# p768lwy3/torecsys

Hardware: AMD Instinct MI355X
Metric: CTR samples/sec fwd+bwd (DeepFM, 39 fields x dim 64) (higher is better)
Workload: dtype bf16; 1 GPU; BASELINE.json configs[1]: DeepFM 39 Criteo-shaped fields, MLP [400,400,400], 1000000 total rows, embed_dim 64, batch 65536, uniform indices, uniform field sizes; global_batch=65536, rows=1000000, parallelism=single, microbatches=1, optimizer=none, hipgraph=True, hipgraph_input_sets=1, hipgraph_steps_per_replay=4, fused_lookup_fm=True

## Files before the change

### include/trs_abi.h

```cpp
#ifndef TRS_ABI_H_
#define TRS_ABI_H_

#include <stddef.h>
#include <stdint.h>

#ifdef __cplusplus
extern "C" {
#endif

#define TRS_ABI_VERSION 3

enum { TRS_F32 = 0, TRS_BF16 = 1 };
enum { TRS_I64 = 0, TRS_I32 = 1 };
enum {
  TRS_OK = 0,
  TRS_EINVAL = -1,
  TRS_EDTYPE = -2,
  TRS_ESHAPE = -3,
  TRS_EALIGN = -4,
  TRS_ELAUNCH = -5,
  TRS_EWORKSPACE = -6
};

typedef void* trs_stream_t;
// ... 25 lines not shown
                       int32_t* err_flag, trs_stream_t stream);

size_t trs_scatter_workspace_bytes(int64_t BN, int32_t N, int32_t E, int32_t dtype);
int trs_scatter_rows(const void* g_rows, int64_t g_rows_batch_stride, const void* g_fm, int32_t g_fm_cols,
                     const float* fm_sum, const void* table, const int32_t* row_start,
                     const int32_t* perm, int64_t BN, int64_t V, int32_t E, int32_t N, int32_t dtype,
                     int64_t padding_row, void* grad_table, void* workspace, size_t ws_bytes,
                     trs_stream_t stream);

int trs_scatter_rows_first(const void* g_rows, int64_t g_rows_batch_stride, const void* g_fm, int32_t g_fm_cols,
                           const float* fm_sum,
                           const void* table, const int32_t* row_start, const int32_t* perm, int64_t BN, int64_t V,
                           int32_t E, int32_t N, int32_t dtype, int64_t padding_row, void* grad_table,
                           const void* g_first, void* grad_first, void* workspace, size_t ws_bytes,
                           trs_stream_t stream);

#define TRS_OPT_ROWWISE 16
int trs_scatter_rows_update(const void* g_rows, int64_t g_rows_batch_stride, const void* g_fm, int32_t g_fm_cols,
                            const float* fm_sum, void* table, const int32_t* row_start, const int32_t* perm,
                            int64_t BN, int64_t V, int32_t E, int32_t N, int32_t dtype, int64_t padding_row,
                            int32_t optimizer, float lr, const float* lr_dev, float eps, float beta1, float beta2,
                            float* state, float* state2, void* workspace, size_t ws_bytes, trs_stream_t stream);

int trs_scatter_rows_update_mapped(const void* g_rows, void* table, const int32_t* row_map, const int32_t* row_start,
                                   const int32_t* perm, int64_t K, int64_t U, int64_t V, int32_t E, int32_t dtype,
                                   int32_t optimizer, float lr, const float* lr_dev, float eps, float beta1, float beta2,
                                   float* state, float* state2, void* workspace, size_t ws_bytes, trs_stream_t stream);

int trs_adam_step_size(int64_t* step, const float* lr_dev, double beta1, double beta2, float* step_size_dev,
                       trs_stream_t stream);
// ... 438 lines not shown
```

### torecsys_amd/_abi.py

```python
from __future__ import annotations

import ctypes
import os
import threading
from ctypes import c_char_p, c_int32, c_int64, c_size_t, c_void_p

import torch

_HERE = os.path.dirname(os.path.abspath(__file__))
LIB_PATH = os.environ.get("TRS_LIB_PATH") or os.path.join(_HERE, "libtrs_hip.so")

TRS_F32, TRS_BF16 = 0, 1
TRS_I64, TRS_I32 = 0, 1

_P, _I32, _I64, _SZ, _F32 = c_void_p, c_int32, c_int64, c_size_t, ctypes.c_float

_OPTIMIZER_TAIL = [_I32, _F32, _P, _F32, _F32, _F32, _P, _P, _P, _SZ, _P]

SIGNATURES = {
    "trs_version": (c_int32, []),
    "trs_last_error_string": (c_char_p, []),
    "trs_rowdot_fwd": (c_int32, [_P, _P, _P, _I64, _I32, _I32, _P, _P]),
    "trs_rowdot_bwd_workspace_bytes": (_SZ, [_I64, _I32]),
    "trs_rowdot_bwd": (c_int32, [_P, _P, _P, _I64, _I32, _I32, _P, _P, _P, _P, _SZ, _P]),
# ... 53 lines not shown
    "trs_rows_gemm": (c_int32, [_P, _I64, _I32, _P, _I32, _I32, _I32, _P, _P, _SZ, _P]),
    "trs_afm_bwd_workspace_bytes": (_SZ, [_I64, _I32, _I32, _I32]),
    "trs_pack_columns": (c_int32, [_P, _P, _I32, _I32, _I64, _P, _I32, _P]),
    "trs_mark_timestamp": (c_int32, [_P, _I32, _P]),
    "trs_wall_clock_khz": (_I64, []),
    "trs_gather_rows": (c_int32, [_P, _I64, _I32, _I32, _P, _I32, _P, _I64, _I32, _P, _P, _P]),
    "trs_gather_rows_tables": (c_int32, [_P, _P, _I32, _I32, _P, _I32, _I64, _I32, _P, _P, _P]),
    "trs_fa_gather_rows": (c_int32, [_P, _I64, _I32, _I32, _P, _I32, _P, _I64, _I32, _P, _P, _P]),
    "trs_csr_workspace_bytes": (_SZ, [_I64, _I64]),
    "trs_csr_build": (c_int32, [_P, _I32, _P, _I64, _I32, _I64, _P, _P, _P, _SZ, _P, _P]),
    "trs_csr_build_skip": (c_int32, [_P, _I32, _P, _I64, _I32, _I64, _I64, _P, _P, _P, _SZ, _P, _P]),
    "trs_scatter_workspace_bytes": (_SZ, [_I64, _I32, _I32, _I32]),
    "trs_scatter_rows": (c_int32, [_P, _I64, _P, _I32, _P, _P, _P, _P, _I64, _I64, _I32, _I32, _I32, _I64, _P, _P, _SZ, _P]),
    "trs_scatter_rows_first": (c_int32, [_P, _I64, _P, _I32, _P, _P, _P, _P, _I64, _I64, _I32, _I32, _I32, _I64, _P, _P, _P, _P,
                                         _SZ, _P]),
    "trs_scatter_rows_update": (c_int32, [_P, _I64, _P, _I32, _P, _P, _P, _P, _I64, _I64, _I32, _I32, _I32, _I64,
                                          *_OPTIMIZER_TAIL]),
    "trs_scatter_rows_update_mapped": (c_int32, [_P, _P, _P, _P, _P, _I64, _I64, _I64, _I32, _I32, *_OPTIMIZER_TAIL]),
    "trs_adam_step_size": (c_int32, [_P, _P, ctypes.c_double, ctypes.c_double, _P, _P]),
    "trs_compact_rows_slots": (_I64, [_I64]),
    "trs_compact_rows": (c_int32, [_P, _I64, _P, _I64, _P, _P]),
    "trs_compact_rows_dense_workspace_bytes": (_SZ, [_I64]),
    "trs_compact_rows_dense": (c_int32, [_P, _I64, _P, _P, _P, _SZ, _P]),
    "trs_embed_fm": (c_int32, [_P, _I64, _I32, _I32, _P, _I32, _P, _I64, _I32, _P, _P, _P, _P, _P, _P, _P]),
    "trs_embed_fm_fields": (c_int32, [_P, _I64, _I32, _I32, _P, _I32, _P, _I64, _I32, _P, _P, _P, _P, _P, _P, _P]),
    "trs_bag_pool_fwd": (c_int32, [_P, _I64, _I32, _I32, _P, _I32, _I64, _I32, _I32, _P, _P, _P, _P]),
    "trs_scatter_argmax_workspace_bytes": (_SZ, [_I64, _I32]),
    "trs_scatter_rows_argmax": (c_int32, [_P, _P, _P, _P, _I64, _I64, _I32, _I32, _I32, _I64, _P, _P, _SZ, _P]),
    "trs_bag_pool_masked_fwd": (c_int32, [_P, _I64, _I32, _I32, _P, _I32, _I64, _I32, _I32, _I64, _P, _P, _P, _P, _P, _P]),
    "trs_scatter_weighted_workspace_bytes": (_SZ, [_I64, _I32]),
# ... 330 lines not shown
```

### torecsys_amd/csrc/scatter.hip

```cpp
#include <algorithm>

#include "trs_common.hpp"

namespace trs {

constexpr int SCAN_THREADS = 256;
constexpr int SCAN_ITEMS = 16;
constexpr int SCAN_TILE = SCAN_THREADS * SCAN_ITEMS;
constexpr int LONG_ROW = 64;
constexpr int LONG_ROW_ELEM = 32;
constexpr int LONG_CHUNK = 256;
constexpr int ELEM_SPLIT = 2048;

template <typename IdxT, bool SKIP = false>
__global__ __launch_bounds__(256) void csr_count_kernel(const IdxT* __restrict__ idx,
                                                        const int64_t* __restrict__ offsets, int64_t BN, int N,
                                                        int64_t V, int32_t* __restrict__ count,
                                                        int32_t* __restrict__ slot, int32_t* __restrict__ err_flag,
                                                        const int32_t* __restrict__ gate, int64_t skip_row = -1) {
  constexpr int U = 4;
  if (gate != nullptr && *gate == 0) return;
  const unsigned n_items = (unsigned)BN, uN = (unsigned)N;
  const unsigned stride = gridDim.x * blockDim.x;
  for (unsigned p0 = blockIdx.x * blockDim.x + threadIdx.x; p0 < n_items; p0 += stride * U) {
// ... 546 lines not shown
            } else {
#pragma unroll
              for (int k = 0; k < VE; ++k) gsum[k] += gf[k];
            }
          } else {
#pragma unroll
            for (int k = 0; k < VE; ++k) acc[k] += gf[k];
          }
        }
      }
    }
  }
}

template <typename T, int LOG2L, bool HAS_G, bool HAS_FM, bool HAS_F1 = false, bool SCAL = false, int CHF = 2,
          bool RW = false>
__global__ __launch_bounds__(256) void scatter_rows_group_kernel(
    const uint4* __restrict__ g_rows, const uint4* __restrict__ g_fm, const float* __restrict__ fm_sum,
    const uint4* __restrict__ table, const int32_t* __restrict__ row_start, const int32_t* __restrict__ perm,
    int64_t V, int N, int64_t gbs, int64_t padding_row, uint4* __restrict__ grad,
    int32_t* __restrict__ long_rows , RowSink sink, FmSrc fs, const T* __restrict__ g_first = nullptr,
    T* __restrict__ grad_first = nullptr) {
  constexpr int L = 1 << LOG2L;
  constexpr int VE = Vec16<T>::VE;
  const int lane_v = threadIdx.x & (L - 1);
  const int64_t groups = ((int64_t)gridDim.x * blockDim.x) >> LOG2L;
  int64_t r = ((int64_t)blockIdx.x * blockDim.x + threadIdx.x) >> LOG2L;
  int nbeg = 0, nend = 0;
  if (r < V) { nbeg = row_start[r]; nend = row_start[r + 1]; }
  for (; r < V; r += groups) {
    const int beg = nbeg, end = nend;
// ... 15 lines not shown
      continue;
    }
    float f1 = 0.f;
    if (r != padding_row) {
      accumulate_bucket<T, LOG2L, HAS_G, HAS_FM, (HAS_FM ? CHF : 4), HAS_F1, SCAL>(acc, gsum, g_rows, g_fm, fm_sum, perm, beg,
                                                                                end, 1, N, gbs, lane_v, fs, g_first, &f1);
      if (HAS_FM && fm_sum != nullptr && end > beg) {
        float w[VE];
        Vec16<T>::unpack(wraw, w);
#pragma unroll
        for (int k = 0; k < VE; ++k) acc[k] = fmaf(-w[k], gsum[SCAL ? 0 : k], acc[k]);
      }
    }
    sink_vec<T, RW, LOG2L>(sink, grad, sink_row(sink, r) * L + lane_v, acc, end > beg && r != padding_row);
    if (HAS_F1 && lane_v == 0) grad_first[r] = from_f32<T>(f1);
  }
}

template <typename T, int LOG2L, bool HAS_G, bool RW = false>
__global__ __launch_bounds__(256, 8) void scatter_rows_fm1_kernel(
    const uint4* __restrict__ g_rows, const uint4* __restrict__ tg, const T* __restrict__ g1,
    const uint4* __restrict__ table, const int32_t* __restrict__ row_start, const int32_t* __restrict__ perm, int V,
    unsigned N, unsigned rcpN , int padding_row, uint4* __restrict__ grad,
    int32_t* __restrict__ long_rows , RowSink sink) {
  constexpr int L = 1 << LOG2L;
  constexpr int VE = Vec16<T>::VE;
  constexpr int CH = 2;
  const unsigned lane_v = threadIdx.x & (L - 1);
  const int groups = (int)(((int64_t)gridDim.x * blockDim.x) >> LOG2L);
  int r = (int)(((int64_t)blockIdx.x * blockDim.x + threadIdx.x) >> LOG2L);
  int nbeg = 0, nend = 0;
  if (r < V) { nbeg = row_start[r]; nend = row_start[r + 1]; }
  for (; r < V; r += groups) {
    const int beg = nbeg, end = nend;
    if (r + groups < V) { nbeg = row_start[r + groups]; nend = row_start[r + groups + 1]; }
    const uint4 wraw = table[(unsigned)r * L + lane_v];
    float acc[VE], gsum = 0.f;
#pragma unroll
    for (int k = 0; k < VE; ++k) acc[k] = 0.f;
// ... 39 lines not shown
          if (HAS_G) Vec16<T>::unpack(gv[c], x);
          Vec16<T>::unpack(tv[c], t);
#pragma unroll
          for (int k = 0; k < VE; ++k) acc[k] += HAS_G ? x[k] + t[k] : t[k];
          gsum += gs[c];
        }
      }
      if (end > beg) {
        float w[VE];
        Vec16<T>::unpack(wraw, w);
#pragma unroll
        for (int k = 0; k < VE; ++k) acc[k] = fmaf(-w[k], gsum, acc[k]);
      }
    }
    sink_vec<T, RW, LOG2L>(sink, grad, sink_row(sink, r) * L + lane_v, acc, end > beg && live);
  }
}

template <typename T>
__global__ __launch_bounds__(256) void scatter_first_long_kernel(const T* __restrict__ g_first,
                                                                 const int32_t* __restrict__ row_start,
                                                                 const int32_t* __restrict__ perm,
                                                                 const int32_t* __restrict__ long_rows,
                                                                 T* __restrict__ grad_first) {
  const int nlong = long_rows[0];
  const int lane = threadIdx.x & 63;
  const int wid = (blockIdx.x * blockDim.x + threadIdx.x) >> 6, nwaves = (gridDim.x * blockDim.x) >> 6;
  for (int i = wid; i < nlong; i += nwaves) {
    if (long_rows[2 + 2 * i] != 0) continue;
    const int64_t r = long_rows[1 + 2 * i];
// ... 1 lines not shown
    float acc = 0.f;
    constexpr int U = 4;
    for (int q = beg + lane; q < end; q += 64 * U) {
      int pp[U];
#pragma unroll
      for (int u = 0; u < U; ++u) pp[u] = (q + 64 * u) < end ? perm[q + 64 * u] : -1;
#pragma unroll
      for (int u = 0; u < U; ++u)
        if (pp[u] >= 0) acc += to_f32(g_first[pp[u]]);
    }
    acc = group_sum_down<64>(acc);
    if (lane == 0) grad_first[r] = from_f32<T>(acc);
  }
}

template <typename T, int LOG2L, bool HAS_G, bool HAS_FM, bool SCAL = false, bool RW = false>
__global__ __launch_bounds__(256) void scatter_long_rows_kernel(
    const uint4* __restrict__ g_rows, const uint4* __restrict__ g_fm, const float* __restrict__ fm_sum,
    const uint4* __restrict__ table, const int32_t* __restrict__ row_start, const int32_t* __restrict__ perm, int N,
    int64_t gbs, uint4* __restrict__ grad, const int32_t* __restrict__ long_rows, float* __restrict__ scratch,
    RowSink sink, FmSrc fs) {
  constexpr int L = 1 << LOG2L;
  constexpr int VE = Vec16<T>::VE;
  constexpr int G = 64 / L;
  const int lane = threadIdx.x & 63;
  const int lane_v = lane & (L - 1);
  const int grp = lane >> LOG2L;
  const int nlong = long_rows[0];
  const int waves = gridDim.x * (blockDim.x >> 6);
  for (int i = blockIdx.x * (blockDim.x >> 6) + (threadIdx.x >> 6); i < nlong; i += waves) {
    const int64_t r = long_rows[1 + 2 * i];
    const int c = long_rows[2 + 2 * i];
    const int rbeg = row_start[r], rend = row_start[r + 1];
    const int beg = rbeg + c * LONG_CHUNK, end = rend < beg + LONG_CHUNK ? rend : beg + LONG_CHUNK;
    const bool single = rend - rbeg <= LONG_CHUNK;
    float acc[VE], gsum[VE];
// ... 9 lines not shown
      for (int k = 0; k < (SCAL ? 1 : VE); ++k) gsum[k] += __shfl_xor(gsum[k], m, 64);
    }
    if (SCAL) {
#pragma unroll
      for (int k = 1; k < VE; ++k) gsum[k] = gsum[0];
    }
    if (grp == 0) {
      if (single) {
        if (HAS_FM && fm_sum != nullptr) {
          float w[VE];
          Vec16<T>::unpack(table[r * L + lane_v], w);
#pragma unroll
          for (int k = 0; k < VE; ++k) acc[k] = fmaf(-w[k], gsum[k], acc[k]);
        }
        sink_vec<T, RW, LOG2L>(sink, grad, sink_row(sink, r) * L + lane_v, acc, true);
      } else {
        float* sa = scratch + ((size_t)i * 2) * (L * VE) + lane_v * VE;
#pragma unroll
        for (int k = 0; k < VE; ++k) { sa[k] = acc[k]; sa[L * VE + k] = gsum[k]; }
      }
    }
  }
}

template <typename T, int LOG2L, bool HAS_FM, bool RW = false>
__global__ __launch_bounds__(256) void scatter_long_rows_finish_kernel(
    const float* __restrict__ fm_sum, const uint4* __restrict__ table, const int32_t* __restrict__ row_start,
    uint4* __restrict__ grad, const int32_t* __restrict__ long_rows, const float* __restrict__ scratch, RowSink sink) {
  constexpr int L = 1 << LOG2L;
  constexpr int VE = Vec16<T>::VE;
  const int lane_v = threadIdx.x & (L - 1);
  const int nlong = long_rows[0];
  const int groups = (gridDim.x * blockDim.x) >> LOG2L;
  for (int i = (blockIdx.x * blockDim.x + threadIdx.x) >> LOG2L; i < nlong; i += groups) {
    if (long_rows[2 + 2 * i] != 0) continue;
    const int64_t r = long_rows[1 + 2 * i];
    const int len = row_start[r + 1] - row_start[r];
    if (len <= LONG_CHUNK) continue;
    const int nch = (len + LONG_CHUNK - 1) / LONG_CHUNK;
    float acc[VE], gsum[VE];
#pragma unroll
    for (int k = 0; k < VE; ++k) { acc[k] = 0.f; gsum[k] = 0.f; }
    constexpr int U = 8;
// ... 15 lines not shown
          gsum[4 * k] += vg[u][k].x; gsum[4 * k + 1] += vg[u][k].y; gsum[4 * k + 2] += vg[u][k].z; gsum[4 * k + 3] += vg[u][k].w;
        }
    }
    for (; c < nch; ++c) {
      const float* sa = scratch + ((size_t)(i + c) * 2) * (L * VE) + lane_v * VE;
#pragma unroll
      for (int k = 0; k < VE; ++k) { acc[k] += sa[k]; gsum[k] += sa[L * VE + k]; }
    }
    if (HAS_FM && fm_sum != nullptr) {
      float w[VE];
      Vec16<T>::unpack(table[r * L + lane_v], w);
#pragma unroll
      for (int k = 0; k < VE; ++k) acc[k] = fmaf(-w[k], gsum[k], acc[k]);
    }
    sink_vec<T, RW, LOG2L>(sink, grad, sink_row(sink, r) * L + lane_v, acc, true);
  }
}

template <typename T>
__global__ __launch_bounds__(256) void build_tg_kernel(const uint4* __restrict__ g_fm, const float* __restrict__ fm_sum,
                                                       uint4* __restrict__ tg, int64_t B, int L,
                                                       int32_t* __restrict__ zero_a, int32_t* __restrict__ zero_b) {
  constexpr int VE = Vec16<T>::VE;
  if (zero_a != nullptr && blockIdx.x == 0 && threadIdx.x == 0) { *zero_a = 0; *zero_b = 0; }
  const int64_t total = B * L, stride = (int64_t)gridDim.x * blockDim.x;
  for (int64_t t = (int64_t)blockIdx.x * blockDim.x + threadIdx.x; t < total; t += stride) {
    const int64_t b = t / L;
    const int lv = (int)(t - b * L);
    const uint4 gv = g_fm[t];
    float g[VE], o[VE];
// ... 182 lines not shown
struct WalkJob {
  const void* g_rows = nullptr;
  int64_t gbs = 0;
  const void* g_fm = nullptr;
  int g_fm_cols = 0;
  const float* fm_sum = nullptr;
  const void* table = nullptr;
  const int32_t* row_start = nullptr;
  const int32_t* perm = nullptr;
  int64_t B = 0, V = 0;
  int E = 0, N = 0;
  int64_t padding_row = -1;
  void* out = nullptr;
  const void* g_first = nullptr;
  void* grad_first = nullptr;
  int32_t* long_rows = nullptr;
  bool zero_in_build = false;
  int32_t* split_count = nullptr;
  void* tg = nullptr;
  float* scratch = nullptr;
  RowSink sink = GRAD_SINK;
  hipStream_t s = nullptr;
  const char* who = "scatter_rows";
};

template <typename T, int LOG2L, bool RW>
static void scatter_group_launch(const WalkJob& j) {
  const int L = 1 << LOG2L;
  hipStream_t s = j.s;
  FmSrc fs{nullptr, nullptr, 0, 0};
// ... 5 lines not shown
      uint4* gvec = (uint4*)j.tg + j.B * L;
      hipLaunchKernelGGL((build_tg1_kernel<T>), dim3(stream_grid(j.B * L, 256, 4096)), dim3(256), 0, s,
                         (const T*)j.g_fm, j.fm_sum, (uint4*)j.tg, gvec, j.B, L, zero_a, j.split_count);
      fs = FmSrc{(const uint4*)j.tg, gvec, L, 1};
      fs.g1 = j.g_fm;
      scal = j.g_first == nullptr;
    } else {
      hipLaunchKernelGGL((build_tg_kernel<T>), dim3(stream_grid(j.B * L, 256, 4096)), dim3(256), 0, s,
                         (const uint4*)j.g_fm, j.fm_sum, (uint4*)j.tg, j.B, L, zero_a, j.split_count);
      fs = FmSrc{(const uint4*)j.tg, (const uint4*)j.tg + L, 2 * L, 2 * L};
    }
    fm = j.tg;
  }
  const int grid = stream_grid(j.V * L, 256, 256 * 32);
  const bool hg = j.g_rows != nullptr, hf = fm != nullptr;
#define TRS_SC_TAIL(HG, HF, SC)                                                                                 \
  do {                                                                                                          \
    hipLaunchKernelGGL((scatter_long_rows_kernel<T, LOG2L, HG, HF, SC, RW>), dim3(2048), dim3(256), 0, s,            \
                       (const uint4*)j.g_rows, (const uint4*)fm, j.fm_sum, (const uint4*)j.table, j.row_start,  \
                       j.perm, j.N, j.gbs, (uint4*)j.out, j.long_rows, j.scratch, j.sink, fs);                  \
    hipLaunchKernelGGL((scatter_long_rows_finish_kernel<T, LOG2L, HF, RW>), dim3(64), dim3(256), 0, s, j.fm_sum,    \
                       (const uint4*)j.table, j.row_start, (uint4*)j.out, j.long_rows, j.scratch, j.sink);      \
  } while (0)
#define TRS_SC(HG, HF)                                                                                          \
  do {                                                                                                          \
    if (j.g_first != nullptr)                                                                                   \
      hipLaunchKernelGGL((scatter_rows_group_kernel<T, LOG2L, HG, HF, true>), dim3(grid), dim3(256), 0, s,       \
                         (const uint4*)j.g_rows, (const uint4*)fm, j.fm_sum, (const uint4*)j.table, j.row_start, \
                         j.perm, j.V, j.N, j.gbs, j.padding_row, (uint4*)j.out, j.long_rows, j.sink, fs,        \
                         (const T*)j.g_first, (T*)j.grad_first);                                                \
    else                                                                                                        \
      hipLaunchKernelGGL((scatter_rows_group_kernel<T, LOG2L, HG, HF, false, false, 2, RW>), dim3(grid), dim3(256), 0, s,             \
                         (const uint4*)j.g_rows, (const uint4*)fm, j.fm_sum, (const uint4*)j.table, j.row_start, \
                         j.perm, j.V, j.N, j.gbs, j.padding_row, (uint4*)j.out, j.long_rows, j.sink, fs);       \
    TRS_SC_TAIL(HG, HF, false);                                                                                 \
  } while (0)
#define TRS_SCS(HG, CHF_)                                                                                       \
  do {                                                                                                          \
    hipLaunchKernelGGL((scatter_rows_group_kernel<T, LOG2L, HG, true, false, true, CHF_, RW>), dim3(grid), dim3(256), 0, s, \
                       (const uint4*)j.g_rows, (const uint4*)fm, j.fm_sum, (const uint4*)j.table, j.row_start,  \
                       j.perm, j.V, j.N, j.gbs, j.padding_row, (uint4*)j.out, j.long_rows, j.sink, fs);         \
    TRS_SC_TAIL(HG, true, true);                                                                                \
  } while (0)
  const bool lean = scal && (j.B * j.N) * (int64_t)L < ((int64_t)1 << 31) && j.V * (int64_t)L < ((int64_t)1 << 31) &&
                    j.N >= 2 && (j.B * j.N) * (int64_t)j.N < ((int64_t)1 << 32) && j.gbs == j.N;
  if (lean) {
    const unsigned rcpN = (unsigned)((((uint64_t)1 << 32) + (unsigned)j.N - 1) / (unsigned)j.N);
    if (hg)
      hipLaunchKernelGGL((scatter_rows_fm1_kernel<T, LOG2L, true, RW>), dim3(grid), dim3(256), 0, s, (const uint4*)j.g_rows,
                         (const uint4*)j.tg, (const T*)fs.g1, (const uint4*)j.table, j.row_start, j.perm, (int)j.V,
                         (unsigned)j.N, rcpN, (int)j.padding_row, (uint4*)j.out, j.long_rows, j.sink);
    else
      hipLaunchKernelGGL((scatter_rows_fm1_kernel<T, LOG2L, false, RW>), dim3(grid), dim3(256), 0, s, (const uint4*)j.g_rows,
                         (const uint4*)j.tg, (const T*)fs.g1, (const uint4*)j.table, j.row_start, j.perm, (int)j.V,
                         (unsigned)j.N, rcpN, (int)j.padding_row, (uint4*)j.out, j.long_rows, j.sink);
    if (hg) TRS_SC_TAIL(true, true, true);
    else TRS_SC_TAIL(false, true, true);
  } else if (scal) {
    if (hg) TRS_SCS(true, 2);
    else TRS_SCS(false, 2);
  } else if (hg && hf) TRS_SC(true, true);
  else if (hg) TRS_SC(true, false);
  else TRS_SC(false, true);
#undef TRS_SC
#undef TRS_SCS
#undef TRS_SC_TAIL
  if (j.g_first != nullptr)
    hipLaunchKernelGGL((scatter_first_long_kernel<T>), dim3(64), dim3(256), 0, s, (const T*)j.g_first, j.row_start,
                       j.perm, j.long_rows, (T*)j.grad_first);
}

static int walk_lanes(const WalkJob& j, int elem_bytes) {
  const int lg = log2_lanes(j.E * elem_bytes);
  const bool scal = j.g_fm_cols == 1 && j.E > 1 && j.fm_sum != nullptr;
  const bool al = aligned16(j.g_rows) && (scal || aligned16(j.g_fm)) && aligned16(j.table) && aligned16(j.out) &&
                  aligned16(j.fm_sum);
  return al ? lg : -1;
}

template <typename T>
// ... 173 lines not shown
  TRS_REQUIRE(j.g_rows || j.g_fm, TRS_EINVAL, "scatter_rows: need g_rows and/or g_fm");
  TRS_REQUIRE((j.fm_sum == nullptr) || (j.g_fm && j.table), TRS_EINVAL, "scatter_rows: fm_sum needs g_fm and table");
  TRS_REQUIRE(j.g_fm == nullptr || j.g_fm_cols == j.E || (j.g_fm_cols == 1 && j.fm_sum != nullptr), TRS_EINVAL,
              "scatter_rows: g_fm_cols %d (E = %d full rows, or 1 = constant along E with fm_sum)", j.g_fm_cols, j.E);
  if (j.gbs <= 0) j.gbs = j.N;
  TRS_REQUIRE(j.gbs >= j.N, TRS_EINVAL, "scatter_rows: g_rows_batch_stride %lld < N", (long long)j.gbs);
  TRS_REQUIRE(j.V > 0 && j.E > 0 && j.N > 0 && BN >= 0, TRS_EINVAL, "scatter_rows: bad size");
  TRS_REQUIRE(dtype == TRS_F32 || dtype == TRS_BF16, TRS_EDTYPE, "scatter_rows: dtype %d", dtype);
  TRS_REQUIRE(ws_bytes >= trs_scatter_workspace_bytes(BN, j.N, j.E, dtype), TRS_EWORKSPACE,
              "scatter_rows: workspace %zu < %zu", ws_bytes, trs_scatter_workspace_bytes(BN, j.N, j.E, dtype));
  TRS_REQUIRE(BN % j.N == 0, TRS_EINVAL, "scatter_rows: B*N=%lld not a multiple of N=%d", (long long)BN, j.N);
  const int lg = walk_lanes(j, dtype_size(dtype));
  TRS_REQUIRE(j.sink.mode != 4 || lg >= 0, TRS_ESHAPE,
              "%s: row-wise Adagrad needs rows of 1, 2, 4 .. 64 whole 16-byte vectors behind 16-byte aligned pointers "
              "(E = %d, %d bytes per value)", j.who, j.E, dtype_size(dtype));
  j.B = BN / j.N;
  j.long_rows = (int32_t*)workspace;
  j.tg = (char*)workspace + long_row_queue_bytes(BN);
  j.scratch = (float*)((char*)j.tg + align_up((size_t)j.B * 2 * j.E * dtype_size(dtype), 256));
  j.split_count = j.long_rows + 1 + (BN / LONG_ROW_ELEM + 2);
  j.zero_in_build = lg >= 0 && j.g_fm != nullptr && j.fm_sum != nullptr;
  if (!j.zero_in_build) hipLaunchKernelGGL(zero_two_i32_kernel, dim3(1), dim3(64), 0, j.s, j.long_rows, j.split_count);
  return dtype == TRS_F32 ? scatter_launch<float>(j, lg) : scatter_launch<bf16_t>(j, lg);
}

extern "C" int trs_scatter_rows_first(const void* g_rows, int64_t g_rows_batch_stride, const void* g_fm, int32_t g_fm_cols,
                                      const float* fm_sum, const void* table, const int32_t* row_start,
                                      const int32_t* perm, int64_t BN, int64_t V, int32_t E, int32_t N, int32_t dtype,
                                      int64_t padding_row, void* grad_table, const void* g_first, void* grad_first,
                                      void* workspace, size_t ws_bytes, trs_stream_t stream) {
  TRS_REQUIRE(g_first && grad_first, TRS_EINVAL, "scatter_rows_first: NULL first-order pointer");
  return scatter_rows_impl(WalkJob{.g_rows = g_rows, .gbs = g_rows_batch_stride, .g_fm = g_fm, .g_fm_cols = g_fm_cols,
                                   .fm_sum = fm_sum, .table = table, .row_start = row_start, .perm = perm, .V = V, .E = E,
                                   .N = N, .padding_row = padding_row, .out = grad_table, .g_first = g_first,
                                   .grad_first = grad_first, .sink = GRAD_SINK, .s = (hipStream_t)stream},
                           BN, dtype, workspace, ws_bytes);
}

extern "C" int trs_scatter_rows(const void* g_rows, int64_t g_rows_batch_stride, const void* g_fm, int32_t g_fm_cols,
                                const float* fm_sum,
                                const void* table, const int32_t* row_start, const int32_t* perm, int64_t BN, int64_t V,
                                int32_t E, int32_t N, int32_t dtype, int64_t padding_row, void* grad_table,
                                void* workspace, size_t ws_bytes, trs_stream_t stream) {
  return scatter_rows_impl(WalkJob{.g_rows = g_rows, .gbs = g_rows_batch_stride, .g_fm = g_fm, .g_fm_cols = g_fm_cols,
                                   .fm_sum = fm_sum, .table = table, .row_start = row_start, .perm = perm, .V = V, .E = E,
                                   .N = N, .padding_row = padding_row, .out = grad_table, .sink = GRAD_SINK,
                                   .s = (hipStream_t)stream},
                           BN, dtype, workspace, ws_bytes);
}

// ... 76 lines not shown
```

### torecsys_amd/functional.py

```python
from __future__ import annotations

import ctypes
import os
from typing import List, Optional, Sequence, Tuple

import torch
from torch.autograd import Function
from torch.autograd.function import once_differentiable

from . import _abi
from ._abi import call, index_dtype_code, ptr, require_device, size_query, stream_ptr, value_dtype_code

CHECK_INDICES = os.environ.get("TRS_CHECK_INDICES", "0") not in ("", "0")


def _as_index(idx: torch.Tensor) -> torch.Tensor:
    idx = idx.rename(None) if idx.has_names() else idx
    if idx.dtype not in (torch.int64, torch.int32):
        if idx.dtype.is_floating_point or idx.dtype == torch.bool:
            raise TypeError(f"indices must be an integer tensor, got {idx.dtype}")
        idx = idx.long()
    return idx.contiguous()


# ... 267 lines not shown
    return grad


def scatter_rows_first(rb: RowBuckets, like_table: torch.Tensor, like_first: torch.Tensor, g_first: torch.Tensor,
                       g_rows: Optional[torch.Tensor] = None, g_bcast: Optional[torch.Tensor] = None,
                       fm_sum: Optional[torch.Tensor] = None, padding_row: int = -1
                       ) -> Tuple[torch.Tensor, torch.Tensor]:
    V, E = like_table.shape
    grad = torch.empty_like(like_table)
    gfirst = torch.empty_like(like_first)
    ws_bytes = size_query("trs_scatter_workspace_bytes", rb.BN, rb.N, E, value_dtype_code(like_table))
    ws = torch.empty(ws_bytes, dtype=torch.uint8, device=like_table.device)
    call("trs_scatter_rows_first", ptr(g_rows), 0, ptr(g_bcast), _bcast_cols(g_bcast, E), ptr(fm_sum),
         ptr(like_table if fm_sum is not None else None), ptr(rb.row_start), ptr(rb.perm), rb.BN, V, E, rb.N,
         value_dtype_code(like_table), padding_row, ptr(grad), ptr(g_first), ptr(gfirst), ptr(ws), ws_bytes, stream_ptr())
    return grad, gfirst


def _adam_step_dev(opt, table: torch.Tensor, key) -> torch.Tensor:
    step, step_size = opt.step_tensors(table, key)
    call("trs_adam_step_size", ptr(step), ptr(opt.lr_tensor(table.device)), float(opt.beta1), float(opt.beta2),
         ptr(step_size), stream_ptr())
    return step_size


TRS_OPT_ROWWISE = 16


def _sink_args(opt, table: torch.Tensor, key, operands=()):
    capturable = getattr(opt, "capturable", False)
# ... 876 lines not shown
    if idx.dim() != 2:
        raise ValueError(f"indices must be (B, N), got shape {tuple(idx.shape)}")
    if padding_idx is not None and padding_idx < 0:
        padding_idx = weight.shape[0] + padding_idx
    emb, fm, first = _EmbedFM.apply(weight, idx, offsets, first_weight, want_emb, opt, False, padding_idx)
    return (emb if want_emb else None), fm, (first if first_weight is not None else None)


def embed_fm_fields(weight: torch.Tensor, first_weight: torch.Tensor, idx: torch.Tensor,
                    offsets: Optional[torch.Tensor] = None, opt=None
                    ) -> Tuple[torch.Tensor, torch.Tensor, torch.Tensor]:
    idx = _as_index(idx)
    if idx.dim() != 2:
        raise ValueError(f"indices must be (B, N), got shape {tuple(idx.shape)}")
    return _EmbedFM.apply(weight, idx, offsets, first_weight, True, opt, True)


class _FMLayer(Function):
    @staticmethod
    def forward(ctx, x):
        require_device(x)
        x = x.contiguous()
        B, N, E = x.shape
        fm = torch.empty(B, E, dtype=x.dtype, device=x.device)
        fm_sum = torch.empty(B, E, dtype=torch.float32, device=x.device)
        call("trs_fm_fwd", ptr(x), B, N, E, value_dtype_code(x), ptr(fm), ptr(fm_sum), stream_ptr())
        ctx.save_for_backward(x, fm_sum)
        return fm

    @staticmethod
# ... 2540 lines not shown
```

### torecsys_amd/inputs.py

```python
from __future__ import annotations

import os
from collections import namedtuple
from typing import Dict, List, Optional, Union

import torch
import torch.nn as nn

from . import functional as F_


def _strip(t: torch.Tensor) -> torch.Tensor:
    return t.rename(None) if t.has_names() else t


def _check_embedding_kwargs(kwargs: dict):
    if kwargs.get("max_norm") is not None:
        raise NotImplementedError("torecsys_amd: nn.Embedding(max_norm=...) is not supported")
    if kwargs.get("scale_grad_by_freq"):
        raise NotImplementedError("torecsys_amd: nn.Embedding(scale_grad_by_freq=True) is not supported")
    if kwargs.get("sparse"):
        raise NotImplementedError("torecsys_amd: nn.Embedding(sparse=True) is not supported (dense gradient only)")


# ... 464 lines not shown
        self.num_fields = num_fields
        self.transforms = transforms
        self.length = 1

    def forward(self, inputs: torch.Tensor) -> torch.Tensor:
        inputs = _strip(inputs)
        if inputs.dim() == 2:
            inputs = inputs.unsqueeze(dim=-1)
        if self.transforms:
            inputs = self.transforms(inputs)
        inputs.names = ('B', 'N', 'E',)
        return inputs


PAIR_FIRST_ORDER = os.environ.get("TRS_PAIR_FIRST_ORDER", "0") == "1"


def _on_hip(t: torch.Tensor) -> bool:
    return t.is_cuda


STACKED_ONE_LAUNCH = os.environ.get("TRS_STACKED_ONE_LAUNCH", "1") not in ("", "0")
LOOKUP_STREAMS = int(os.environ.get("TRS_LOOKUP_STREAMS", "1") or 0)
_SIDE_LOOKUPS = (SingleIndexEmbedding, MultiIndicesEmbedding, MultiIndicesFieldAwareEmbedding)


class Inputs(BaseInput):

    def __init__(self, schema: Union[Dict[str, nn.Module], None]):
        super().__init__()
        self.schema = schema if schema is not None else {}
        for k, emb_fn in self.schema.items():
            self.add_module(k, emb_fn)
        self.length = None

    def _first_order_partner(self, key: str) -> Optional[str]:
        a = self.schema[key]
        if not PAIR_FIRST_ORDER:
            return None
        if type(a) is not MultiIndicesEmbedding or not a.fuse_fm or a.flatten or a.padding_idx is not None:
            return None
        if getattr(a, 'fused_optimizer', None) is not None or not a.embedding.weight.is_cuda:
            return None
        wa = a.embedding.weight
        if (wa.shape[1] * wa.element_size()) % 16 != 0:
            return None
        for k, f in self.schema.items():
            if k == key or type(f) is not MultiIndicesEmbedding:
                continue
            if (f.embed_size != 1 or f.flatten or f.fuse_fm or f.padding_idx is not None
                    or getattr(f, 'fused_optimizer', None) is not None):
                continue
            wf = f.embedding.weight
            if (tuple(f.schema.inputs) != tuple(a.schema.inputs) or wf.shape[0] != wa.shape[0] or wf.dtype != wa.dtype
                    or wf.device != wa.device or wf.requires_grad != wa.requires_grad):
                continue
            same = self._same_layout.get((key, k))
# ... 71 lines not shown
                else:
                    cols = [v.unsqueeze(-1) if v.dim() == 1 else v for v in raw]
                    inp = cols[0] if len(cols) == 1 else torch.cat(cols, dim=1)
                packed[names] = inp
            args[k] = [inp]
            if emb_fn.__class__.__name__ in ('SequenceIndicesEmbedding', 'SequenceIndexEmbedding'):
                args[k].append(inputs[emb_fn.schema.lengths])
            elif emb_fn.__class__.__name__ in ('RaggedListIndicesEmbedding', 'RaggedMultiListIndicesEmbedding'):
                args[k].append(inputs[emb_fn.schema.offsets])
                args[k].append(None if emb_fn.schema.weights is None else inputs[emb_fn.schema.weights])
            elif getattr(emb_fn.schema, 'weights', None) is not None:
                args[k].append(inputs[emb_fn.schema.weights])
        side_keys, first_lookup = [], True
        for k in args:
            emb_fn = self.schema[k]
            plain = (type(emb_fn) in _SIDE_LOOKUPS and k not in partner.values()
                     and isinstance(args[k][0], torch.Tensor) and args[k][0].is_cuda)
            if plain and not first_lookup and LOOKUP_STREAMS:
                side_keys.append(k)
            first_lookup = first_lookup and not plain
        joins = []
        def side_lookups():
            for k in side_keys:
                emb_fn, idx_t = self.schema[k], args[k][0]
                out, ev, side = F_.run_on_side(idx_t.device, "lookup", lambda: emb_fn(idx_t))
                idx_t.record_stream(side)
                joins.append((ev, out))
                outputs[k] = out

        with F_.defer_prefetch():
            if LOOKUP_STREAMS == 2:
                side_lookups()
            for k in args:
                if k in outputs or k in side_keys:
                    continue
                emb_fn, inp_args = self.schema[k], args[k]
                feat_key = next((f for f, w in partner.items() if w == k), None)
                if feat_key is not None:
                    feat_fn = self.schema[feat_key]
                    idx = inp_args[0].rename(None) if inp_args[0].has_names() else inp_args[0]
                    if idx.dim() != 2 or idx.shape[1] != emb_fn.offsets.numel():
                        raise ValueError(f'inputs must be (B, {emb_fn.offsets.numel()}), got {tuple(idx.shape)}')
                    out, fm, first = F_.embed_fm_fields(emb_fn.embedding.weight, feat_fn.embedding.weight, idx,
                                                        emb_fn.offsets)
                    out._trs_fused_fm = (fm, out._version)
                    out.names = ('B', 'N', 'E',)
                    first.names = ('B', 'N', 'E',)
                    outputs[k] = out
                    outputs[feat_key] = first
                else:
                    outputs[k] = emb_fn(*inp_args)
            if LOOKUP_STREAMS != 2:
                side_lookups()
        if joins:
            main = F_._abi.current_stream_of(joins[0][1].device)
            for ev, out in joins:
                main.wait_event(ev)
                extra = [t[0] for t in (getattr(out, a, None) for a in ('_trs_fused_fm', '_trs_fused_ipn')) if t is not None]
                for t in [out] + extra:
# ... 22 lines not shown
```

Before: 67.40 million samples/s.

## Pair first-order table with FM embedding and fuse its gradient into the scatter walk

Adds a new default-on path (TRS_PAIR_FIRST_ORDER_WALK) that pairs the first-order linear table with the FM embedding lookup. The forward runs the first-order gather on a side stream, and the backward uses one scatter walk that writes both the embedding gradient and the first-order gradient. It relies on the FM output gradient and the first-order gradient being the same broadcast column, so the per-row sum already computed for the FM term also serves as the first-order gradient. This removes a separate scatter pass over the first-order table. In exchange it adds template variants and a narrower eligibility check that falls back when the gradients do not share storage.

```diff
diff --git a/include/trs_abi.h b/include/trs_abi.h
--- a/include/trs_abi.h
+++ b/include/trs_abi.h
@@ -63,6 +63,12 @@
                            int32_t E, int32_t N, int32_t dtype, int64_t padding_row, void* grad_table,
                            const void* g_first, void* grad_first, void* workspace, size_t ws_bytes,
                            trs_stream_t stream);
+
+int trs_scatter_rows_first_same(const void* g_rows, int64_t g_rows_batch_stride, const void* g_fm, int32_t g_fm_cols,
+                                const float* fm_sum, const void* table, const int32_t* row_start, const int32_t* perm,
+                                int64_t BN, int64_t V, int32_t E, int32_t N, int32_t dtype, int64_t padding_row,
+                                void* grad_table, void* grad_first, void* workspace, size_t ws_bytes,
+                                trs_stream_t stream);
 
 #define TRS_OPT_ROWWISE 16
 int trs_scatter_rows_update(const void* g_rows, int64_t g_rows_batch_stride, const void* g_fm, int32_t g_fm_cols,
diff --git a/torecsys_amd/_abi.py b/torecsys_amd/_abi.py
--- a/torecsys_amd/_abi.py
+++ b/torecsys_amd/_abi.py
@@ -91,6 +91,8 @@
     "trs_scatter_rows": (c_int32, [_P, _I64, _P, _I32, _P, _P, _P, _P, _I64, _I64, _I32, _I32, _I32, _I64, _P, _P, _SZ, _P]),
     "trs_scatter_rows_first": (c_int32, [_P, _I64, _P, _I32, _P, _P, _P, _P, _I64, _I64, _I32, _I32, _I32, _I64, _P, _P, _P, _P,
                                          _SZ, _P]),
+    "trs_scatter_rows_first_same": (c_int32, [_P, _I64, _P, _I32, _P, _P, _P, _P, _I64, _I64, _I32, _I32, _I32, _I64, _P, _P, _P,
+                                              _SZ, _P]),
     "trs_scatter_rows_update": (c_int32, [_P, _I64, _P, _I32, _P, _P, _P, _P, _I64, _I64, _I32, _I32, _I32, _I64,
                                           *_OPTIMIZER_TAIL]),
     "trs_scatter_rows_update_mapped": (c_int32, [_P, _P, _P, _P, _P, _I64, _I64, _I64, _I32, _I32, *_OPTIMIZER_TAIL]),
diff --git a/torecsys_amd/csrc/scatter.hip b/torecsys_amd/csrc/scatter.hip
--- a/torecsys_amd/csrc/scatter.hip
+++ b/torecsys_amd/csrc/scatter.hip
@@ -584,7 +584,7 @@
 }
 
 template <typename T, int LOG2L, bool HAS_G, bool HAS_FM, bool HAS_F1 = false, bool SCAL = false, int CHF = 2,
-          bool RW = false>
+          bool RW = false, bool F1S = false>
 __global__ __launch_bounds__(256) void scatter_rows_group_kernel(
     const uint4* __restrict__ g_rows, const uint4* __restrict__ g_fm, const float* __restrict__ fm_sum,
     const uint4* __restrict__ table, const int32_t* __restrict__ row_start, const int32_t* __restrict__ perm,
@@ -630,15 +630,16 @@
     }
     sink_vec<T, RW, LOG2L>(sink, grad, sink_row(sink, r) * L + lane_v, acc, end > beg && r != padding_row);
     if (HAS_F1 && lane_v == 0) grad_first[r] = from_f32<T>(f1);
-  }
-}
-
-template <typename T, int LOG2L, bool HAS_G, bool RW = false>
+    if (F1S && lane_v == 0) grad_first[r] = from_f32<T>(gsum[0]);
+  }
+}
+
+template <typename T, int LOG2L, bool HAS_G, bool RW = false, bool F1S = false>
 __global__ __launch_bounds__(256, 8) void scatter_rows_fm1_kernel(
     const uint4* __restrict__ g_rows, const uint4* __restrict__ tg, const T* __restrict__ g1,
     const uint4* __restrict__ table, const int32_t* __restrict__ row_start, const int32_t* __restrict__ perm, int V,
     unsigned N, unsigned rcpN , int padding_row, uint4* __restrict__ grad,
-    int32_t* __restrict__ long_rows , RowSink sink) {
+    int32_t* __restrict__ long_rows , RowSink sink, T* __restrict__ grad_first = nullptr) {
   constexpr int L = 1 << LOG2L;
   constexpr int VE = Vec16<T>::VE;
   constexpr int CH = 2;
@@ -708,6 +709,7 @@
       }
     }
     sink_vec<T, RW, LOG2L>(sink, grad, sink_row(sink, r) * L + lane_v, acc, end > beg && live);
+    if (F1S && lane_v == 0) grad_first[r] = from_f32<T>(gsum);
   }
 }
 
@@ -739,12 +741,12 @@
   }
 }
 
-template <typename T, int LOG2L, bool HAS_G, bool HAS_FM, bool SCAL = false, bool RW = false>
+template <typename T, int LOG2L, bool HAS_G, bool HAS_FM, bool SCAL = false, bool RW = false, bool F1S = false>
 __global__ __launch_bounds__(256) void scatter_long_rows_kernel(
     const uint4* __restrict__ g_rows, const uint4* __restrict__ g_fm, const float* __restrict__ fm_sum,
     const uint4* __restrict__ table, const int32_t* __restrict__ row_start, const int32_t* __restrict__ perm, int N,
     int64_t gbs, uint4* __restrict__ grad, const int32_t* __restrict__ long_rows, float* __restrict__ scratch,
-    RowSink sink, FmSrc fs) {
+    RowSink sink, FmSrc fs, T* __restrict__ grad_first = nullptr) {
   constexpr int L = 1 << LOG2L;
   constexpr int VE = Vec16<T>::VE;
   constexpr int G = 64 / L;
@@ -784,6 +786,7 @@
           for (int k = 0; k < VE; ++k) acc[k] = fmaf(-w[k], gsum[k], acc[k]);
         }
         sink_vec<T, RW, LOG2L>(sink, grad, sink_row(sink, r) * L + lane_v, acc, true);
+        if (F1S && lane_v == 0) grad_first[r] = from_f32<T>(gsum[0]);
       } else {
         float* sa = scratch + ((size_t)i * 2) * (L * VE) + lane_v * VE;
 #pragma unroll
@@ -793,10 +796,11 @@
   }
 }
 
-template <typename T, int LOG2L, bool HAS_FM, bool RW = false>
+template <typename T, int LOG2L, bool HAS_FM, bool RW = false, bool F1S = false>
 __global__ __launch_bounds__(256) void scatter_long_rows_finish_kernel(
     const float* __restrict__ fm_sum, const uint4* __restrict__ table, const int32_t* __restrict__ row_start,
-    uint4* __restrict__ grad, const int32_t* __restrict__ long_rows, const float* __restrict__ scratch, RowSink sink) {
+    uint4* __restrict__ grad, const int32_t* __restrict__ long_rows, const float* __restrict__ scratch, RowSink sink,
+    T* __restrict__ grad_first = nullptr) {
   constexpr int L = 1 << LOG2L;
   constexpr int VE = Vec16<T>::VE;
   const int lane_v = threadIdx.x & (L - 1);
@@ -842,6 +846,7 @@
       for (int k = 0; k < VE; ++k) acc[k] = fmaf(-w[k], gsum[k], acc[k]);
     }
     sink_vec<T, RW, LOG2L>(sink, grad, sink_row(sink, r) * L + lane_v, acc, true);
+    if (F1S && lane_v == 0) grad_first[r] = from_f32<T>(gsum[0]);
   }
 }
 
@@ -1054,6 +1059,7 @@
   void* out = nullptr;
   const void* g_first = nullptr;
   void* grad_first = nullptr;
+  bool first_same = false;
   int32_t* long_rows = nullptr;
   bool zero_in_build = false;
   int32_t* split_count = nullptr;
@@ -1089,13 +1095,15 @@
   }
   const int grid = stream_grid(j.V * L, 256, 256 * 32);
   const bool hg = j.g_rows != nullptr, hf = fm != nullptr;
-#define TRS_SC_TAIL(HG, HF, SC)                                                                                 \
+#define TRS_SC_TAIL(HG, HF, SC, F1)                                                                             \
   do {                                                                                                          \
-    hipLaunchKernelGGL((scatter_long_rows_kernel<T, LOG2L, HG, HF, SC, RW>), dim3(2048), dim3(256), 0, s,            \
+    hipLaunchKernelGGL((scatter_long_rows_kernel<T, LOG2L, HG, HF, SC, RW, F1>), dim3(2048), dim3(256), 0, s,   \
                        (const uint4*)j.g_rows, (const uint4*)fm, j.fm_sum, (const uint4*)j.table, j.row_start,  \
-                       j.perm, j.N, j.gbs, (uint4*)j.out, j.long_rows, j.scratch, j.sink, fs);                  \
-    hipLaunchKernelGGL((scatter_long_rows_finish_kernel<T, LOG2L, HF, RW>), dim3(64), dim3(256), 0, s, j.fm_sum,    \
-                       (const uint4*)j.table, j.row_start, (uint4*)j.out, j.long_rows, j.scratch, j.sink);      \
+                       j.perm, j.N, j.gbs, (uint4*)j.out, j.long_rows, j.scratch, j.sink, fs,                   \
+                       (T*)j.grad_first);                                                                       \
+    hipLaunchKernelGGL((scatter_long_rows_finish_kernel<T, LOG2L, HF, RW, F1>), dim3(64), dim3(256), 0, s,      \
+                       j.fm_sum, (const uint4*)j.table, j.row_start, (uint4*)j.out, j.long_rows, j.scratch,     \
+                       j.sink, (T*)j.grad_first);                                                               \
   } while (0)
 #define TRS_SC(HG, HF)                                                                                          \
   do {                                                                                                          \
@@ -1108,37 +1116,52 @@
       hipLaunchKernelGGL((scatter_rows_group_kernel<T, LOG2L, HG, HF, false, false, 2, RW>), dim3(grid), dim3(256), 0, s,             \
                          (const uint4*)j.g_rows, (const uint4*)fm, j.fm_sum, (const uint4*)j.table, j.row_start, \
                          j.perm, j.V, j.N, j.gbs, j.padding_row, (uint4*)j.out, j.long_rows, j.sink, fs);       \
-    TRS_SC_TAIL(HG, HF, false);                                                                                 \
+    TRS_SC_TAIL(HG, HF, false, false);                                                                          \
   } while (0)
-#define TRS_SCS(HG, CHF_)                                                                                       \
+#define TRS_SCS(HG, CHF_, F1)                                                                                   \
   do {                                                                                                          \
-    hipLaunchKernelGGL((scatter_rows_group_kernel<T, LOG2L, HG, true, false, true, CHF_, RW>), dim3(grid), dim3(256), 0, s, \
-                       (const uint4*)j.g_rows, (const uint4*)fm, j.fm_sum, (const uint4*)j.table, j.row_start,  \
-                       j.perm, j.V, j.N, j.gbs, j.padding_row, (uint4*)j.out, j.long_rows, j.sink, fs);         \
-    TRS_SC_TAIL(HG, true, true);                                                                                \
+    hipLaunchKernelGGL((scatter_rows_group_kernel<T, LOG2L, HG, true, false, true, CHF_, RW, F1>), dim3(grid),  \
+                       dim3(256), 0, s, (const uint4*)j.g_rows, (const uint4*)fm, j.fm_sum,                     \
+                       (const uint4*)j.table, j.row_start, j.perm, j.V, j.N, j.gbs, j.padding_row,              \
+                       (uint4*)j.out, j.long_rows, j.sink, fs, (const T*)nullptr, (T*)j.grad_first);            \
+    TRS_SC_TAIL(HG, true, true, F1);                                                                            \
+  } while (0)
+#define TRS_FM1(HG, F1)                                                                                         \
+  do {                                                                                                          \
+    hipLaunchKernelGGL((scatter_rows_fm1_kernel<T, LOG2L, HG, RW, F1>), dim3(grid), dim3(256), 0, s,            \
+                       (const uint4*)j.g_rows, (const uint4*)j.tg, (const T*)fs.g1, (const uint4*)j.table,      \
+                       j.row_start, j.perm, (int)j.V, (unsigned)j.N, rcpN, (int)j.padding_row, (uint4*)j.out,   \
+                       j.long_rows, j.sink, (T*)j.grad_first);                                                  \
+    TRS_SC_TAIL(HG, true, true, F1);                                                                            \
   } while (0)
   const bool lean = scal && (j.B * j.N) * (int64_t)L < ((int64_t)1 << 31) && j.V * (int64_t)L < ((int64_t)1 << 31) &&
                     j.N >= 2 && (j.B * j.N) * (int64_t)j.N < ((int64_t)1 << 32) && j.gbs == j.N;
-  if (lean) {
+  bool first_same = false;
+  if constexpr (!RW) first_same = j.first_same;
+  if (first_same) {
+    if constexpr (!RW) {
+      if (lean) {
+        const unsigned rcpN = (unsigned)((((uint64_t)1 << 32) + (unsigned)j.N - 1) / (unsigned)j.N);
+        if (hg) TRS_FM1(true, true);
+        else TRS_FM1(false, true);
+      } else {
+        if (hg) TRS_SCS(true, 2, true);
+        else TRS_SCS(false, 2, true);
+      }
+    }
+  } else if (lean) {
     const unsigned rcpN = (unsigned)((((uint64_t)1 << 32) + (unsigned)j.N - 1) / (unsigned)j.N);
-    if (hg)
-      hipLaunchKernelGGL((scatter_rows_fm1_kernel<T, LOG2L, true, RW>), dim3(grid), dim3(256), 0, s, (const uint4*)j.g_rows,
-                         (const uint4*)j.tg, (const T*)fs.g1, (const uint4*)j.table, j.row_start, j.perm, (int)j.V,
-                         (unsigned)j.N, rcpN, (int)j.padding_row, (uint4*)j.out, j.long_rows, j.sink);
-    else
-      hipLaunchKernelGGL((scatter_rows_fm1_kernel<T, LOG2L, false, RW>), dim3(grid), dim3(256), 0, s, (const uint4*)j.g_rows,
-                         (const uint4*)j.tg, (const T*)fs.g1, (const uint4*)j.table, j.row_start, j.perm, (int)j.V,
-                         (unsigned)j.N, rcpN, (int)j.padding_row, (uint4*)j.out, j.long_rows, j.sink);
-    if (hg) TRS_SC_TAIL(true, true, true);
-    else TRS_SC_TAIL(false, true, true);
+    if (hg) TRS_FM1(true, false);
+    else TRS_FM1(false, false);
   } else if (scal) {
-    if (hg) TRS_SCS(true, 2);
-    else TRS_SCS(false, 2);
+    if (hg) TRS_SCS(true, 2, false);
+    else TRS_SCS(false, 2, false);
   } else if (hg && hf) TRS_SC(true, true);
   else if (hg) TRS_SC(true, false);
   else TRS_SC(false, true);
 #undef TRS_SC
 #undef TRS_SCS
+#undef TRS_FM1
 #undef TRS_SC_TAIL
   if (j.g_first != nullptr)
     hipLaunchKernelGGL((scatter_first_long_kernel<T>), dim3(64), dim3(256), 0, s, (const T*)j.g_first, j.row_start,
@@ -1342,6 +1365,9 @@
   TRS_REQUIRE(j.sink.mode != 4 || lg >= 0, TRS_ESHAPE,
               "%s: row-wise Adagrad needs rows of 1, 2, 4 .. 64 whole 16-byte vectors behind 16-byte aligned pointers "
               "(E = %d, %d bytes per value)", j.who, j.E, dtype_size(dtype));
+  TRS_REQUIRE(!j.first_same || lg >= 0, TRS_ESHAPE,
+              "%s: needs rows of 1, 2, 4 .. 64 whole 16-byte vectors behind 16-byte aligned pointers (E = %d, %d bytes "
+              "per value): the element walk has no companion form", j.who, j.E, dtype_size(dtype));
   j.B = BN / j.N;
   j.long_rows = (int32_t*)workspace;
   j.tg = (char*)workspace + long_row_queue_bytes(BN);
@@ -1362,6 +1388,26 @@
                                    .fm_sum = fm_sum, .table = table, .row_start = row_start, .perm = perm, .V = V, .E = E,
                                    .N = N, .padding_row = padding_row, .out = grad_table, .g_first = g_first,
                                    .grad_first = grad_first, .sink = GRAD_SINK, .s = (hipStream_t)stream},
+                           BN, dtype, workspace, ws_bytes);
+}
+
+extern "C" int trs_scatter_rows_first_same(const void* g_rows, int64_t g_rows_batch_stride, const void* g_fm,
+                                           int32_t g_fm_cols, const float* fm_sum, const void* table,
+                                           const int32_t* row_start, const int32_t* perm, int64_t BN, int64_t V, int32_t E,
+                                           int32_t N, int32_t dtype, int64_t padding_row, void* grad_table,
+                                           void* grad_first, void* workspace, size_t ws_bytes, trs_stream_t stream) {
+  const char* who = "scatter_rows_first_same";
+  TRS_REQUIRE(grad_first, TRS_EINVAL, "%s: NULL grad_first", who);
+  TRS_REQUIRE(g_fm && fm_sum && table, TRS_EINVAL, "%s: needs the FM term (g_fm, fm_sum, table)", who);
+  TRS_REQUIRE(g_fm_cols == 1, TRS_EINVAL,
+              "%s: g_fm_cols %d: the companion gradient is the sum of ONE FM scalar per sample (g_fm_cols = 1)", who,
+              g_fm_cols);
+  TRS_REQUIRE(padding_row < 0, TRS_EINVAL, "%s: no padding row (the companion table has none), got %lld", who,
+              (long long)padding_row);
+  return scatter_rows_impl(WalkJob{.g_rows = g_rows, .gbs = g_rows_batch_stride, .g_fm = g_fm, .g_fm_cols = g_fm_cols,
+                                   .fm_sum = fm_sum, .table = table, .row_start = row_start, .perm = perm, .V = V, .E = E,
+                                   .N = N, .padding_row = -1, .out = grad_table, .grad_first = grad_first,
+                                   .first_same = true, .sink = GRAD_SINK, .s = (hipStream_t)stream, .who = who},
                            BN, dtype, workspace, ws_bytes);
 }
 
diff --git a/torecsys_amd/functional.py b/torecsys_amd/functional.py
--- a/torecsys_amd/functional.py
+++ b/torecsys_amd/functional.py
@@ -305,6 +305,20 @@
     call("trs_scatter_rows_first", ptr(g_rows), 0, ptr(g_bcast), _bcast_cols(g_bcast, E), ptr(fm_sum),
          ptr(like_table if fm_sum is not None else None), ptr(rb.row_start), ptr(rb.perm), rb.BN, V, E, rb.N,
          value_dtype_code(like_table), padding_row, ptr(grad), ptr(g_first), ptr(gfirst), ptr(ws), ws_bytes, stream_ptr())
+    return grad, gfirst
+
+
+def scatter_rows_first_same(rb: RowBuckets, like_table: torch.Tensor, like_first: torch.Tensor, g_col: torch.Tensor,
+                            fm_sum: torch.Tensor, g_rows: Optional[torch.Tensor] = None
+                            ) -> Tuple[torch.Tensor, torch.Tensor]:
+    V, E = like_table.shape
+    grad = torch.empty(V, E, dtype=like_table.dtype, device=like_table.device)
+    gfirst = torch.empty_like(like_first)
+    ws_bytes = size_query("trs_scatter_workspace_bytes", rb.BN, rb.N, E, value_dtype_code(like_table))
+    ws = torch.empty(ws_bytes, dtype=torch.uint8, device=like_table.device)
+    call("trs_scatter_rows_first_same", ptr(g_rows), 0, ptr(g_col), 1, ptr(fm_sum), ptr(like_table), ptr(rb.row_start),
+         ptr(rb.perm), rb.BN, V, E, rb.N, value_dtype_code(like_table), -1, ptr(grad), ptr(gfirst), ptr(ws), ws_bytes,
+         stream_ptr())
     return grad, gfirst
 
 
@@ -1211,6 +1225,113 @@
     if idx.dim() != 2:
         raise ValueError(f"indices must be (B, N), got shape {tuple(idx.shape)}")
     return _EmbedFM.apply(weight, idx, offsets, first_weight, True, opt, True)
+
+
+def _same_column(g_fm: torch.Tensor, g_first: torch.Tensor) -> bool:
+    if g_fm.dim() != 2 or g_first.dim() != 3 or g_first.shape[2] != 1 or g_fm.shape[0] != g_first.shape[0]:
+        return False
+    if (g_fm.shape[1] > 1 and g_fm.stride(1) != 0) or (g_first.shape[1] > 1 and g_first.stride(1) != 0):
+        return False
+    return (g_fm.dtype == g_first.dtype and g_fm.data_ptr() == g_first.data_ptr()
+            and (g_fm.shape[0] <= 1 or g_fm.stride(0) == g_first.stride(0)))
+
+
+class _EmbedFMFirst(Function):
+
+    @staticmethod
+    def forward(ctx, weight, idx, offsets, first_weight, opt=None, side=1):
+        require_device(weight, idx, offsets, first_weight)
+        B, N = idx.shape
+        V, E = weight.shape
+        if first_weight.dtype != weight.dtype or first_weight.numel() != V:
+            raise ValueError("first-order table must be (V,1) with the embedding table's dtype")
+        w, fw = weight.contiguous(), first_weight.contiguous()
+        dev = w.device
+        flag = _ErrFlag(dev)
+
+        def first_lookup():
+            out = torch.empty(B, N, 1, dtype=fw.dtype, device=dev)
+            call("trs_gather_rows", ptr(fw), V, 1, value_dtype_code(fw), ptr(idx), index_dtype_code(idx), ptr(offsets), B, N,
+                 ptr(out), ptr(flag.t), stream_ptr())
+            return out
+
+        def wide_lookup():
+            emb = torch.empty(B, N, E, dtype=w.dtype, device=dev)
+            fm = torch.empty(B, E, dtype=w.dtype, device=dev)
+            fm_sum = torch.empty(B, E, dtype=torch.float32, device=dev)
+            if PREFETCH_EARLY and (ctx.needs_input_grad[0] or ctx.needs_input_grad[3]):
+                prefetch_row_buckets(idx, offsets, V, now=True)
+            call("trs_embed_fm", ptr(w), V, E, value_dtype_code(w), ptr(idx), index_dtype_code(idx), ptr(offsets), B, N,
+                 ptr(emb), ptr(fm), ptr(fm_sum), None, None, ptr(flag.t), stream_ptr())
+            return emb, fm, fm_sum
+
+        join = None
+        if side == 2:
+            first, ev, st = run_on_side(dev, "lookup", first_lookup)
+            join = (ev, st)
+        emb, fm, fm_sum = wide_lookup()
+        if side == 1:
+            first, ev, st = run_on_side(dev, "lookup", first_lookup)
+            join = (ev, st)
+        elif side != 2:
+            first = first_lookup()
+        if join is not None:
+            main = _abi.current_stream_of(dev)
+            main.wait_event(join[0])
+            first.record_stream(main)
+            idx.record_stream(join[1])
+        flag.check("embed_fm")
+        if ctx.needs_input_grad[0] or ctx.needs_input_grad[3]:
+            prefetch_row_buckets(idx, offsets, V)
+        ctx.save_for_backward(idx, offsets, weight, first_weight, fm_sum)
+        ctx.opt = opt
+        ctx.set_materialize_grads(False)
+        return emb, fm, first
+
+    @staticmethod
+    @once_differentiable
+    def backward(ctx, g_emb, g_fm, g_first):
+        idx, offsets, weight, first_weight, fm_sum = ctx.saved_tensors
+        g_emb, g_fm, g_first = [g.rename(None) if g is not None and g.has_names() else g for g in (g_emb, g_fm, g_first)]
+        _adopt_grads(g_emb, g_fm, g_first)
+        V, E = weight.shape
+        rb = row_buckets(idx, offsets, V)
+        gw = gfw = None
+        need_w, need_f = ctx.needs_input_grad[0], ctx.needs_input_grad[3]
+        if (need_w and need_f and ctx.opt is None and g_fm is not None and g_first is not None
+                and _same_column(g_fm, g_first)):
+            g_rows = g_emb.contiguous() if g_emb is not None else None
+            g_col = _fm_grad_operand(g_fm)
+            if g_col.shape[1] == 1 and _walk_takes_vectors(weight, g_rows, weight, fm_sum):
+                gw, gfw = scatter_rows_first_same(rb, weight, first_weight, g_col, fm_sum, g_rows=g_rows)
+                return gw, None, None, gfw, None, None
+        if need_w:
+            if g_emb is not None or g_fm is not None:
+                gw = _apply_or_grad(rb, weight, ctx.opt, g_rows=g_emb.contiguous() if g_emb is not None else None,
+                                    g_bcast=_fm_grad_operand(g_fm) if g_fm is not None else None,
+                                    fm_sum=fm_sum if g_fm is not None else None)
+            elif ctx.opt is None:
+                gw = torch.zeros_like(weight)
+        if need_f:
+            if g_first is not None:
+                fw2 = first_weight.reshape(V, 1)
+                if g_first.shape[1] > 1 and g_first.stride(1) == 0:
+                    gfw = _apply_or_grad(rb, fw2, ctx.opt, key=first_weight, g_bcast=g_first[:, 0, :].contiguous())
+                else:
+                    gfw = _apply_or_grad(rb, fw2, ctx.opt, key=first_weight, g_rows=g_first.contiguous())
+                gfw = None if gfw is None else gfw.reshape(first_weight.shape)
+            elif ctx.opt is None:
+                gfw = torch.zeros_like(first_weight)
+        return gw, None, None, gfw, None, None
+
+
+def embed_fm_first(weight: torch.Tensor, first_weight: torch.Tensor, idx: torch.Tensor,
+                   offsets: Optional[torch.Tensor] = None, opt=None, side: int = 1
+                   ) -> Tuple[torch.Tensor, torch.Tensor, torch.Tensor]:
+    idx = _as_index(idx)
+    if idx.dim() != 2:
+        raise ValueError(f"indices must be (B, N), got shape {tuple(idx.shape)}")
+    return _EmbedFMFirst.apply(weight, idx, offsets, first_weight, opt, int(side))
 
 
 class _FMLayer(Function):
diff --git a/torecsys_amd/inputs.py b/torecsys_amd/inputs.py
--- a/torecsys_amd/inputs.py
+++ b/torecsys_amd/inputs.py
@@ -502,6 +502,7 @@
 
 
 PAIR_FIRST_ORDER = os.environ.get("TRS_PAIR_FIRST_ORDER", "0") == "1"
+PAIR_FIRST_ORDER_WALK = os.environ.get("TRS_PAIR_FIRST_ORDER_WALK", "1") not in ("", "0")
 
 
 def _on_hip(t: torch.Tensor) -> bool:
@@ -524,11 +525,11 @@
 
     def _first_order_partner(self, key: str) -> Optional[str]:
         a = self.schema[key]
-        if not PAIR_FIRST_ORDER:
+        if not (PAIR_FIRST_ORDER or PAIR_FIRST_ORDER_WALK):
             return None
         if type(a) is not MultiIndicesEmbedding or not a.fuse_fm or a.flatten or a.padding_idx is not None:
             return None
-        if getattr(a, 'fused_optimizer', None) is not None or not a.embedding.weight.is_cuda:
+        if getattr(a, 'fused_optimizer', None) is not None or not _on_hip(a.embedding.weight):
             return None
         wa = a.embedding.weight
         if (wa.shape[1] * wa.element_size()) % 16 != 0:
@@ -630,9 +631,10 @@
         side_keys, first_lookup = [], True
         for k in args:
             emb_fn = self.schema[k]
-            plain = (type(emb_fn) in _SIDE_LOOKUPS and k not in partner.values()
+            served = k in partner.values()
+            plain = (type(emb_fn) in _SIDE_LOOKUPS and not (served and PAIR_FIRST_ORDER)
                      and isinstance(args[k][0], torch.Tensor) and args[k][0].is_cuda)
-            if plain and not first_lookup and LOOKUP_STREAMS:
+            if plain and not first_lookup and LOOKUP_STREAMS and not served:
                 side_keys.append(k)
             first_lookup = first_lookup and not plain
         joins = []
@@ -657,8 +659,12 @@
                     idx = inp_args[0].rename(None) if inp_args[0].has_names() else inp_args[0]
                     if idx.dim() != 2 or idx.shape[1] != emb_fn.offsets.numel():
                         raise ValueError(f'inputs must be (B, {emb_fn.offsets.numel()}), got {tuple(idx.shape)}')
-                    out, fm, first = F_.embed_fm_fields(emb_fn.embedding.weight, feat_fn.embedding.weight, idx,
-                                                        emb_fn.offsets)
+                    if PAIR_FIRST_ORDER:
+                        out, fm, first = F_.embed_fm_fields(emb_fn.embedding.weight, feat_fn.embedding.weight, idx,
+                                                            emb_fn.offsets)
+                    else:
+                        out, fm, first = F_.embed_fm_first(emb_fn.embedding.weight, feat_fn.embedding.weight, idx,
+                                                           emb_fn.offsets, side=LOOKUP_STREAMS)
                     out._trs_fused_fm = (fm, out._version)
                     out.names = ('B', 'N', 'E',)
                     first.names = ('B', 'N', 'E',)
```

Result: no change. 67.86 million samples/s (median of 6 runs) (+0.7%).
